# rlorenzo/facet

Hardware: AMD Instinct MI355X
Metric: images/sec whole-node (TOPIQ+SAMP+CLIP+InsightFace ensemble), 1024² batch (higher is better)
Workload: dtype f32

## Files before the change

facet_amd/csrc/engine.hip:

```cpp
#include "engine.h"
#include "onnx_graph.h"
#include "wino64_maps.h"
#include <algorithm>
#include <cmath>
#include <cstdlib>

namespace fe {

void WeightStore::set(const std::string& name, const float* data, const int64_t* shape, int ndim) {
  HostTensor h;
  h.shape.assign(shape, shape + ndim);
  h.data.assign(data, data + h.numel());
  t_[name] = std::move(h);
}
const HostTensor& WeightStore::get(const std::string& name) const {
  auto it = t_.find(name);
  if (it == t_.end()) throw Error("missing weight tensor '" + name + "'");
  return it->second;
}

float* DeviceWeights::upload(const std::vector<float>& v) {
  void* p = nullptr;
  const size_t b = v.size() * sizeof(float);
  FE_HIP(hipMalloc(&p, b ? b : 16));
// ... 663 lines not shown
}

template <class E>
static void linear_forward_half(Ctx& c, const ConvW& w, const E* x, int ldx, int M, E* y, int ldy, int act, const E* res, int ldr) {
  FE_CHECK(w.wh && w.hprec == PrecOf<E>::value, "linear(2-byte): layer has no weights of the activations' type");
  if (M <= 32 && !res && act != ACT_PRELU && ldx % 4 == 0 && ((uintptr_t)x & 7) == 0) {
    launch_gemm_skinny(x, ldx, (const E*)w.wh, w.KpH, w.scale, w.shift, y, ldy, M, w.Cout, w.CinPadH, act, c.stream);
    c.flops_accum += 2.0 * M * (double)w.Cin * (w.CoutAlg ? w.CoutAlg : w.Cout);
    return;
  }
  TensorT<E> xt = mat_view(x, M, w.CinPadH, ldx), yt = mat_view(y, M, w.Cout, ldy);
  ConvOptsT<E> o; o.act = act;
  TensorT<E> rt;
  if (res) { rt = mat_view(res, M, w.Cout, ldr); o.res = &rt; }
  conv_forward(c, w, xt, yt, o);
}
template <class E>
static void linear_forward_s32_half(Ctx& c, const ConvW& w, const E* x, int ldx, int M, float* y, int ldy, int act, const float* res, int ldr) {
  FE_CHECK(w.wh && w.hprec == PrecOf<E>::value, "linear(2-byte): layer has no weights of the activations' type");
  TensorT<E> xt = mat_view(x, M, w.CinPadH, ldx), yt = mat_view((E*)nullptr, M, w.Cout, 0);
  Tensor y32 = mat_view(y, M, w.Cout, ldy), r32;
  ConvOptsT<E> o; o.act = act; o.y32 = &y32;
  if (res) { r32 = mat_view(res, M, w.Cout, ldr); o.res32 = &r32; }
  conv_forward(c, w, xt, yt, o);
}
void linear_forward_s32(Ctx& c, const ConvW& w, const bf16* x, int ldx, int M, float* y, int ldy, int act, const float* res, int ldr) {
  linear_forward_s32_half<bf16>(c, w, x, ldx, M, y, ldy, act, res, ldr);
}
void linear_forward_s32(Ctx& c, const ConvW& w, const f16* x, int ldx, int M, float* y, int ldy, int act, const float* res, int ldr) {
  linear_forward_s32_half<f16>(c, w, x, ldx, M, y, ldy, act, res, ldr);
}
void linear_forward(Ctx& c, const ConvW& w, const bf16* x, int ldx, int M, bf16* y, int ldy, int act, const bf16* res, int ldr) {
  linear_forward_half<bf16>(c, w, x, ldx, M, y, ldy, act, res, ldr);
}
void linear_forward(Ctx& c, const ConvW& w, const f16* x, int ldx, int M, f16* y, int ldy, int act, const f16* res, int ldr) {
  linear_forward_half<f16>(c, w, x, ldx, M, y, ldy, act, res, ldr);
}
template <class E>
static void linear_forward_f32_half(Ctx& c, const ConvW& w, const E* x, int ldx, int M, float* y, int ldy, int act) {
  FE_CHECK(w.wh && w.hprec == PrecOf<E>::value && act != ACT_PRELU && ldx % 4 == 0 && ((uintptr_t)x & 7) == 0, "linear_f32(2-byte): unsupported layer");
  for (int m0 = 0; m0 < M; m0 += 32) {
    const int mb = std::min(32, M - m0);
    launch_gemm_skinny(x + (size_t)m0 * ldx, ldx, (const E*)w.wh, w.KpH, w.scale, w.shift, y + (size_t)m0 * ldy, ldy, mb, w.Cout, w.CinPadH, act, c.stream);
  }
  c.flops_accum += 2.0 * M * (double)w.Cin * (w.CoutAlg ? w.CoutAlg : w.Cout);
}
void linear_forward_f32(Ctx& c, const ConvW& w, const bf16* x, int ldx, int M, float* y, int ldy, int act) { linear_forward_f32_half<bf16>(c, w, x, ldx, M, y, ldy, act); }
void linear_forward_f32(Ctx& c, const ConvW& w, const f16* x, int ldx, int M, float* y, int ldy, int act) { linear_forward_f32_half<f16>(c, w, x, ldx, M, y, ldy, act); }
void linear_forward_xf32(Ctx& c, const ConvW& w, int prec, const float* x, int ldx, int M, float* y, int ldy, int act) {
  FE_CHECK(w.wh && w.hprec == prec && act != ACT_PRELU && ldx % 4 == 0 && ((uintptr_t)x & 15) == 0, "linear_xf32: unsupported layer");
  for (int m0 = 0; m0 < M; m0 += 32) {
    const int mb = std::min(32, M - m0);
    if (prec == PREC_F16) launch_gemm_skinny(x + (size_t)m0 * ldx, ldx, (const f16*)w.wh, w.KpH, w.scale, w.shift, y + (size_t)m0 * ldy, ldy, mb, w.Cout, w.CinPadH, act, c.stream);
    else launch_gemm_skinny(x + (size_t)m0 * ldx, ldx, (const bf16*)w.wh, w.KpH, w.scale, w.shift, y + (size_t)m0 * ldy, ldy, mb, w.Cout, w.CinPadH, act, c.stream);
  }
  c.flops_accum += 2.0 * M * (double)w.Cin * (w.CoutAlg ? w.CoutAlg : w.Cout);
}

MHAW build_mha(DeviceWeights& dw, const WeightStore& ws, const std::string& prefix, int heads) {
  MHAW m;
  const HostTensor& W = ws.get(prefix + ".in_proj_weight");
  const HostTensor& Bv = ws.get(prefix + ".in_proj_bias");
  const int d = (int)W.shape[1];
  FE_CHECK(W.shape[0] == 3 * d && d % heads == 0 && d % 32 == 0, "mha %s: bad in_proj shape", prefix.c_str());
  m.d = d; m.heads = heads;
  m.q = build_linear_rows(dw, W, nullptr, 0, d);
  m.k = build_linear_rows(dw, W, &Bv, d, d);
  const float sc = 1.0f / std::sqrt((float)(d / heads));
  std::vector<float> qs(d, sc), qb(d);
  for (int i = 0; i < d; ++i) qb[i] = Bv.data[i] * sc;
  m.q.scale = dw.upload(qs);
  m.q.shift = dw.upload(qb);
  std::vector<float> wv(W.data.begin() + (size_t)2 * d * d, W.data.begin() + (size_t)3 * d * d);
  std::vector<float> bv(Bv.data.begin() + 2 * d, Bv.data.begin() + 3 * d);
  m.wv = dw.upload(wv);
  m.bv = dw.upload(bv);
  if (dw.prec != PREC_F32) {
    std::vector<uint16_t> wvh(wv.size());
    for (size_t i = 0; i < wv.size(); ++i) wvh[i] = f32_to_half_bits(wv[i], dw.prec);
    m.wv_h = dw.upload_raw(wvh.data(), wvh.size() * sizeof(uint16_t));
  }
  m.out = build_linear(dw, ws, prefix + ".out_proj", true);
  return m;
}

static void launch_gemm(const ConvParams& p, hipStream_t s) { launch_conv(p, s); }
static void launch_gemm(const ConvParamsH& p, hipStream_t s) { launch_conv_bf16(p, s); }
static void launch_gemm(const ConvParamsT<f16>& p, hipStream_t s) { launch_conv_bf16(p, s); }

template <class T>
static void raw_gemm(Ctx& c, ConvParamsT<T>& p, double flops) {
  constexpr int kalign = sizeof(T) == 2 ? CONV_KALIGN_H : CONV_KALIGN;
  constexpr int valign = 16 / sizeof(T);
  p.N = 1; p.H = 1; p.W = p.M; p.Ho = 1; p.Wo = p.M;
  p.KH = p.KW = 1; p.sh = p.sw = p.dh = p.dw = 1; p.ph = p.pw = 0;
  p.Kp = (p.K + kalign - 1) / kalign * kalign;
  p.Cin = p.K;
  FE_CHECK(p.xs1 % valign == 0 && p.xs2 % valign == 0 && p.ws1 % valign == 0 && p.ws2 % valign == 0, "raw_gemm: batch strides must keep 16-B alignment");
  FE_CHECK(p.ldw == 0 || p.ldw == p.Kp || p.K % kalign == 0, "raw_gemm: K = %d must be a multiple of %d when the B operand is an activation matrix", p.K, kalign);
  hipEvent_t e0 = nullptr, e1 = nullptr;
  if (c.profile) {
    FE_HIP(hipEventCreate(&e0)); FE_HIP(hipEventCreate(&e1));
    FE_HIP(hipEventRecord(e0, c.stream));
  }
  launch_gemm(p, c.stream);
  if (c.profile) {
    FE_HIP(hipEventRecord(e1, c.stream));
    FE_HIP(hipEventSynchronize(e1));
    float ms = 0.f;
    FE_HIP(hipEventElapsedTime(&ms, e0, e1));
    (void)hipEventDestroy(e0); (void)hipEventDestroy(e1);
    char nm[128];
    snprintf(nm, sizeof nm, "%sbgemm x%d M=%d K=%d N=%d", PrecOf<T>::value == PREC_F16 ? "f16 " : (PrecOf<T>::value == PREC_BF16 ? "bf16 " : ""), p.batch > 1 ? p.batch : 1, p.M, p.K, p.Cout);
    c.timings.push_back({nm, flops, 0.0, ms});
  }
  c.flops_accum += flops;
  if (sizeof(T) == 2) c.flops_half += flops;
}

static const float* mha_wv(const MHAW& m, const float*) { return m.wv; }
static const bf16* mha_wv(const MHAW& m, const bf16*) {
  FE_CHECK(m.wv_h && m.q.hprec == PREC_BF16, "mha(bf16): model was not committed under bf16 precision");
  return (const bf16*)m.wv_h;
}
static const f16* mha_wv(const MHAW& m, const f16*) {
  FE_CHECK(m.wv_h && m.q.hprec == PREC_F16, "mha(f16): model was not committed under f16 precision");
  return (const f16*)m.wv_h;
}

void linear_forward_res(Ctx& c, const ConvW& w, const float* x, int ldx, int M, float* y, int ldy, int act, const float* res, int ldr) { linear_forward(c, w, x, ldx, M, y, ldy, act, res, ldr); }
void linear_forward_res(Ctx& c, const ConvW& w, const bf16* x, int ldx, int M, bf16* y, int ldy, int act, const bf16* res, int ldr) { linear_forward(c, w, x, ldx, M, y, ldy, act, res, ldr); }
void linear_forward_res(Ctx& c, const ConvW& w, const f16* x, int ldx, int M, f16* y, int ldy, int act, const f16* res, int ldr) { linear_forward(c, w, x, ldx, M, y, ldy, act, res, ldr); }
void linear_forward_res(Ctx& c, const ConvW& w, const bf16* x, int ldx, int M, float* y, int ldy, int act, const float* res, int ldr) { linear_forward_s32(c, w, x, ldx, M, y, ldy, act, res, ldr); }
void linear_forward_res(Ctx& c, const ConvW& w, const f16* x, int ldx, int M, float* y, int ldy, int act, const float* res, int ldr) { linear_forward_s32(c, w, x, ldx, M, y, ldy, act, res, ldr); }

template <class T, class RT>
void mha_forward(Ctx& c, const MHAW& m, const T* q_in, int ldq, const T* kv_in, int ldkv, int B, int Lq, int Lk,
                 const RT* res, int ldr, RT* y, int ldy, bool causal) {
  constexpr bool half = sizeof(T) == 2;
  const int d = m.d, H = m.heads, hd = d / H;
  const int Lp = (Lk + 31) / 32 * 32;
  const size_t mark = c.arena.mark();
  T* Q = c.arena.array<T>((size_t)B * Lq * d);
  T* K = c.arena.array<T>((size_t)B * Lk * d);
  T* Vt = c.arena.array<T>((size_t)B * d * Lp);
  static const bool no_flash = getenv("FE_NO_FLASH") != nullptr;
  const bool flash = (hd == 64) && (!no_flash || half);
  FE_CHECK(flash || !causal, "causal attention needs the fused kernel (head_dim 64)");
  FE_CHECK(flash || !half, "attention(bf16) needs head_dim 64");
  T* S = flash ? nullptr : c.arena.array<T>((size_t)B * H * Lq * Lp);
  T* O = c.arena.array<T>((size_t)B * Lq * d);
  linear_forward(c, m.q, q_in, ldq, B * Lq, Q, d, ACT_NONE);
  linear_forward(c, m.k, kv_in, ldkv, B * Lk, K, d, ACT_NONE);
  if (Lp != Lk) FE_HIP(hipMemsetAsync(Vt, 0, (size_t)B * d * Lp * sizeof(T), c.stream));
  {
    ConvParamsT<T> p{};
    p.x = mha_wv(m, q_in); p.ldx = d; p.w = kv_in; p.ldw = ldkv; p.y = Vt; p.ldy = Lp;
    p.M = d; p.K = d; p.Cout = Lk;
    p.batch = B; p.nb1 = 1; p.ws2 = (long long)Lk * ldkv; p.ys2 = (long long)d * Lp;
    p.pad_store = half ? 1 : 0;
    raw_gemm(c, p, 2.0 * B * d * (double)d * Lk);
  }
  if (flash) {
    launch_attention(Q, d, K, d, Vt, Lp, m.bv, O, d, B, H, Lq, Lk, d, causal ? 1 : 0, c.stream);
    c.flops_accum += 4.0 * B * H * (double)Lq * Lk * hd;
    if (half) c.flops_half += 4.0 * B * H * (double)Lq * Lk * hd;
  } else if constexpr (!half) {
    {
      ConvParams p{};
      p.x = Q; p.ldx = d; p.w = K; p.ldw = d; p.y = S; p.ldy = Lp;
      p.M = Lq; p.K = hd; p.Cout = Lk;
      p.batch = B * H; p.nb1 = H;
      p.xs1 = hd; p.xs2 = (long long)Lq * d; p.ws1 = hd; p.ws2 = (long long)Lk * d;
      p.ys1 = (long long)Lq * Lp; p.ys2 = (long long)H * Lq * Lp;
      raw_gemm(c, p, 2.0 * B * H * (double)Lq * Lk * hd);
    }
    launch_softmax_rows_pad(S, Lp, B * H * Lq, Lk, c.stream);
    {
      ConvParams p{};
      p.x = S; p.ldx = Lp; p.w = Vt; p.ldw = Lp; p.y = O; p.ldy = d;
      p.shift = m.bv; p.hs1 = hd;
      p.M = Lq; p.K = Lp; p.Cout = hd;
      p.batch = B * H; p.nb1 = H;
      p.xs1 = (long long)Lq * Lp; p.xs2 = (long long)H * Lq * Lp;
      p.ws1 = (long long)hd * Lp; p.ws2 = (long long)d * Lp;
      p.ys1 = hd; p.ys2 = (long long)Lq * d;
      raw_gemm(c, p, 2.0 * B * H * (double)Lq * Lk * hd);
    }
  }
  linear_forward_res(c, m.out, (const T*)O, d, B * Lq, y, ldy, ACT_NONE, res, ldr);
  c.arena.rewind(mark);
}
template void mha_forward<float, float>(Ctx&, const MHAW&, const float*, int, const float*, int, int, int, int, const float*, int, float*, int, bool);
template void mha_forward<bf16, bf16>(Ctx&, const MHAW&, const bf16*, int, const bf16*, int, int, int, int, const bf16*, int, bf16*, int, bool);
template void mha_forward<f16, f16>(Ctx&, const MHAW&, const f16*, int, const f16*, int, int, int, int, const f16*, int, f16*, int, bool);
template void mha_forward<bf16, float>(Ctx&, const MHAW&, const bf16*, int, const bf16*, int, int, int, int, const float*, int, float*, int, bool);
template void mha_forward<f16, float>(Ctx&, const MHAW&, const f16*, int, const f16*, int, int, int, int, const float*, int, float*, int, bool);

}
```

facet_amd/csrc/fe_common.h:

```cpp
#pragma once
#include <hip/hip_runtime.h>
#include "fe_check.h"
#include <cstdint>
#include <cstdio>
#include <atomic>
#include <cstring>
#include <map>
#include <mutex>
#include <stdexcept>
#include <string>
#include <utility>
#include <vector>

namespace fe {


#define FE_HIP(expr)                                                                      \
  do {                                                                                    \
    hipError_t _e = (expr);                                                               \
    if (_e != hipSuccess) {                                                               \
      char _b[512];                                                                       \
      snprintf(_b, sizeof _b, "%s:%d: %s -> %s", __FILE__, __LINE__, #expr,               \
               hipGetErrorString(_e));                                                    \
      throw fe::Error(_b);                                                                \
// ... 163 lines not shown
    return (char*)base_ + a;
  }
  template <class T>
  TensorT<T> tensor_t(int n, int h, int w, int c) {
    TensorT<T> t;
    t.n = n; t.h = h; t.w = w; t.c = c; t.ld = c;
    t.p = (T*)alloc(t.numel() * sizeof(T));
    return t;
  }
  Tensor tensor(int n, int h, int w, int c) { return tensor_t<float>(n, h, w, c); }
  template <class T>
  T* array(size_t count) { return (T*)alloc(count * sizeof(T)); }
 private:
  void* base_ = nullptr;
  size_t cap_ = 0, off_ = 0, high_ = 0;
};

template <class T>
struct ConvParamsT {
  const T* x; int ldx;
  const T* w;
  const float* scale;
  const float* shift;
  const float* slope;
  const T* res; int ldr;
  const T* gate; int ldg;
  T* y; int ldy;
  int N, H, W, Cin, Ho, Wo, Cout;
  int KH, KW, sh, sw, ph, pw, dh, dw;
  int K, Kp, M;
  int act;
  int res_after_act;
  int gate_c1;
  int vec_epi;
  int unit_stride;
  int ldw;
  int batch, nb1;
  long long xs1, xs2, ws1, ws2, ys1, ys2, hs1;
  int buf_ok; unsigned x_span, w_span;
  unsigned y_span, r_span, g_span;
  int variant;
  int cb;
  int pad_store;
  const float* res32; int ldr32;
  float* y32; int ldy32;
  unsigned r32_span, y32_span;
  int a_wrap;
  int split_lo_off;
  int exact_act;
};
using ConvParams = ConvParamsT<float>;
using ConvParamsH = ConvParamsT<bf16>;

struct ConvW {
  float* w = nullptr;
  float* scale = nullptr;
  float* shift = nullptr;
  float* slope = nullptr;
  int Cout = 0, Cin = 0, CinPad = 0, KH = 1, KW = 1, K = 0, Kp = 0;
  int CoutAlg = 0;
  float* wtap = nullptr;
  int wino_m = 0;
  float* wino = nullptr;
  float* wino64 = nullptr;
  float* wstem = nullptr;
  float* wn16 = nullptr;
  int KpT = 0;
  void* wh = nullptr;
  int hprec = 0;
  int KpH = 0, cb = 0, CinPadH = 0;
  void* wtap_h = nullptr;
  int KpTH = 0;
  uint8_t* w8 = nullptr;
  float* w8_scale = nullptr;
};

template <class T>
struct ConvOptsT {
  int sh = 1, sw = 1, ph = 0, pw = 0, dh = 1, dw = 1;
  int act = ACT_NONE;
  const TensorT<T>* res = nullptr;
  int res_after_act = 0;
  const TensorT<T>* gate = nullptr;
  const TensorT<float>* res32 = nullptr;
  const TensorT<float>* y32 = nullptr;
};
using ConvOpts = ConvOptsT<float>;

constexpr int CONV_KALIGN = 32;
constexpr int CONV_KALIGN_H = 64;

void launch_conv(const ConvParams& p, hipStream_t s);
void launch_wino_input(const Tensor& x, int th, int tw, float* V, hipStream_t s);
void launch_wino_output(const float* Mb, const Tensor& y, int th, int tw, const float* scale, const float* shift, int relu, hipStream_t s);
void launch_wino4_input(const Tensor& x, int th, int tw, float* V, hipStream_t s);
void launch_wino4_output(const float* Mb, const Tensor& y, int th, int tw, const float* scale, const float* shift, int act, const float* slope,
                         const Tensor* res, int res_after_act, hipStream_t s);
void launch_wino64(const Tensor& x, const Tensor& y, const float* U, const float* scale, const float* shift, const float* slope, int act,
                   const Tensor* res, int res_after_act, hipStream_t s);
template <class TO>
bool launch_stem(const float* x, int ldx, int N, int H, int W, const float* wstem, const float* scale, const float* shift, const float* slope,
                 int Cout, int k, int stride, int act, TO* y, int ldy, int Ho, int Wo, hipStream_t s);
void launch_conv_narrow(const ConvParams& p, hipStream_t s);
void launch_conv_dma(const ConvParams& p, int tile, hipStream_t s);
void launch_conv_bf16(const ConvParamsH& p, hipStream_t s);
void launch_conv_bf16(const ConvParamsT<f16>& p, hipStream_t s);
template <class T, class Launch>
inline bool conv_split_by_images(const ConvParamsT<T>& p, Launch&& launch) {
  if (p.batch > 1 || p.N <= 1 || (long long)p.N * p.Ho * p.Wo != (long long)p.M) return false;
  const unsigned long long in_img = (unsigned long long)p.H * p.W * p.ldx * sizeof(T);
  unsigned long long out_img = (unsigned long long)p.Ho * p.Wo * (unsigned long long)(p.ldy > p.ldr ? p.ldy : p.ldr) * sizeof(T);
  const unsigned long long out32_img = (unsigned long long)p.Ho * p.Wo * (unsigned long long)(p.ldy32 > p.ldr32 ? p.ldy32 : p.ldr32) * sizeof(float);
  if ((p.y32 || p.res32) && out32_img > out_img) out_img = out32_img;
  const unsigned long long per_img = in_img > out_img ? in_img : out_img;
  constexpr unsigned long long LIMIT = 0xF0000000ull;
  if (per_img >= LIMIT) return false;
  const int ng = (int)(LIMIT / per_img);
  if (ng >= p.N) return false;
  for (int i0 = 0; i0 < p.N; i0 += ng) {
    ConvParamsT<T> q = p;
    const int n = ng < p.N - i0 ? ng : p.N - i0;
    const size_t opix = (size_t)i0 * p.Ho * p.Wo;
    q.N = n; q.M = n * p.Ho * p.Wo;
    q.x = p.x + (size_t)i0 * p.H * p.W * p.ldx;
    if (p.y) q.y = p.y + opix * p.ldy;
    if (p.y32) q.y32 = p.y32 + opix * p.ldy32;
    if (p.res32) q.res32 = p.res32 + opix * p.ldr32;
    if (p.res) q.res = p.res + opix * p.ldr;
    if (p.gate) q.gate = p.gate + opix * p.ldg;
    launch(q);
  }
  return true;
}

double conv_flops(const ConvParams& p);

void launch_u8_to_nhwc4_norm(const uint8_t* src, float* dst, size_t pixels, const float mean[3],
                             const float stdv[3], int bgr, hipStream_t s);
template <class T> void launch_nchw_to_nhwc(const float* src, T* dst, int n, int c, int h, int w, int cpad, hipStream_t s);
template <class T> void launch_nhwc_to_nchw(const T* src, int lds_, float* dst, int n, int c, int h, int w, hipStream_t s);
template <class T> void launch_maxpool(const TensorT<T>& x, const TensorT<T>& y, int k, int stride, int pad, hipStream_t s);
template <class T> void launch_bilinear(const TensorT<T>& x, const TensorT<T>& y, hipStream_t s);
template <class T> void launch_adaptive_avgpool(const TensorT<T>& x, const TensorT<T>& y, hipStream_t s);
void launch_convert(const float* x, bf16* y, size_t n, hipStream_t s);
void launch_convert(const bf16* x, float* y, size_t n, hipStream_t s);
void launch_convert(const float* x, f16* y, size_t n, hipStream_t s);
void launch_convert(const f16* x, float* y, size_t n, hipStream_t s);
void launch_splitk_reduce(const float* part, int splits, int M, int N, const float* scale, const float* shift, const float* slope, int act,
                          const float* res, int ldr, int res_after_act, float* y, int ldy, hipStream_t s);
template <class T>
void launch_tap_gather(const T* z, int ldz, int n, int h, int w, int kh, int kw, int ph, int pw, int dh, int dw,
                       int cout, const float* scale, const float* shift, int act, T* y, int ldy, int ho, int wo,
                       hipStream_t s);
void launch_attention(const float* q, int ldq, const float* k, int ldk, const float* vt, int lp, const float* bv, float* o,
                      int ldo, int B, int H, int Lq, int Lk, int dmodel, int causal, hipStream_t s);
void launch_attention(const bf16* q, int ldq, const bf16* k, int ldk, const bf16* vt, int lp, const float* bv, bf16* o,
                      int ldo, int B, int H, int Lq, int Lk, int dmodel, int causal, hipStream_t s);
void launch_attention(const f16* q, int ldq, const f16* k, int ldk, const f16* vt, int lp, const float* bv, f16* o,
                      int ldo, int B, int H, int Lq, int Lk, int dmodel, int causal, hipStream_t s);
void launch_attention_split(const f16* q, const f16* k, int ld, int lo_off, const f16* vt_hi, const f16* vt_lo, int lp, f16* o, int ldo, int o_lo_off,
                            int B, int H, int Lq, int Lk, int dmodel, hipStream_t s);
template <class TI, class TW, class TO>
void launch_gemm_skinny(const TI* x, int ldx, const TW* w, int ldw, const float* scale, const float* shift, TO* y,
                        int ldy, int M, int N, int K, int act, hipStream_t s);
void launch_sigmoid(const Tensor& x, const Tensor& y, hipStream_t s);
void launch_add(const Tensor& a, const Tensor& b, const Tensor& y, hipStream_t s);
void launch_layernorm_split(const float* x, int ldx, f16* y, int ldy, const float* g, const float* b, int rows, int d, float eps, hipStream_t s);
void launch_split_hi_lo(const float* x, f16* y, size_t rows, int cols, hipStream_t s);
template <class T, class TO>
void launch_layernorm(const T* x, int ldx, TO* y, int ldy, const float* g, const float* b,
                      int rows, int d, float eps, hipStream_t s);
void launch_softmax_rows(float* x, int ld, int rows, int d, hipStream_t s);
void launch_softmax_rows_pad(float* x, int ld, int rows, int d, hipStream_t s);
template <class T>
void launch_add_rows_bcast(T* y, int ldy, const float* pos, int rows, int L, int d, hipStream_t s);

void launch_affine_act(const Tensor& x, const Tensor& y, const float* scale, const float* shift, int act, const float* slope,
                       hipStream_t s);
void launch_binary(const Tensor& a, const Tensor& b, const Tensor& y, int op, int act, hipStream_t s);
void launch_gather_strided(const float* src, float* dst, const long long dims[6], const long long sstr[6], hipStream_t s);
void launch_nearest(const Tensor& x, const Tensor& y, hipStream_t s);
void launch_avgpool(const Tensor& x, const Tensor& y, int k, int stride, int pad, int include_pad, hipStream_t s);
void launch_dwconv(const Tensor& x, const Tensor& y, const float* wt, int kh, int kw, int sh, int sw, int ph, int pw,
                   const float* scale, const float* shift, int act, const float* slope, const Tensor* res, hipStream_t s);

void launch_cv_resize_linear(const uint8_t* src, int n, int h, int w, uint8_t* dst, int ch, int cw, int nh, int nw, const int* xofs,
                             const short* ialpha, const int* yofs, const short* ibeta, int area2, hipStream_t s);
void launch_warp_affine(const uint8_t* src, int h, int w, const int* img_of, const double* Minv, int m, int S, const short* wtab,
                        uint8_t* dst, hipStream_t s);
void launch_swap_rb_u8(const uint8_t* src, uint8_t* dst, size_t pixels, hipStream_t s);
void launch_u8_blob(const uint8_t* src, float* dst, size_t pixels, float mean, float scale, int swap_rb, hipStream_t s);
void launch_scrfd_decode(const float* scores, const float* bbox, const float* kps, int n, int fh, int fw, int A, int K, int stride,
                         float thresh, float det_scale, int level, float* cand, int* counts, int max_cand, hipStream_t s);
void cv_resize_tables(int src, int dst, bool clamp_fx, std::vector<int>& ofs, std::vector<short>& coef);
void cv_warp_weight_table(std::vector<short>& wtab);

constexpr int FE_STATS_COUNT = 264;
size_t stats_accum_bytes(int n);
void launch_image_stats(const uint8_t* bgr, int n, int h, int w, uint8_t* gray, uint8_t* hsv_out, const int* sdiv, const int* hdiv, void* accum,
                        double* out, hipStream_t s);
void cv_hsv_tables(std::vector<int>& sdiv, std::vector<int>& hdiv);
void launch_roi_laplacian(const uint8_t* bgr, int h, int w, const int* img_of, const int* rois, int m, double* out, hipStream_t s);
void launch_canny_map(const uint8_t* d_bgr, int n, int h, int w, int low, int high, uint8_t* d_blur, void* d_grad, void* d_mag, uint8_t* d_map,
                      hipStream_t s);
void launch_canny_map_gray(const uint8_t* d_gray, int n, int h, int w, const int* d_thr, void* d_grad, void* d_mag, uint8_t* d_map, hipStream_t s);
struct ContourScratch {
  int* lab_fg;
  int* lab_bg;
  int* cnt;
  int* strong;
  int* xmin;
  int* xmax;
  int* ymax;
  uint8_t* outer;
  uint8_t* edge;
  int* work;
  int* work_count;
  long long* recs;
  int* rec_count;
  int* error;
};
constexpr int FE_CONTOUR_RECORD = 8;
int contour_work_cap(int h, int w);
size_t contour_scratch_bytes(int nb, int h, int w);
void contour_scratch_carve(ContourScratch& sc, void* base, int nb, int h, int w);
void launch_median_thresholds(const double* d_stats, int n, long long npx, int* d_thr, hipStream_t s);
void launch_external_contours(const uint8_t* d_img, int nb, int h, int w, int candidates, long long min_twice_area, ContourScratch& sc,
                              hipStream_t s);

}
```

facet_amd/csrc/kernels_attn.hip:

```cpp
#include <type_traits>

#include "fe_common.h"

namespace fe {

template <class T>
struct AttnParamsH {
  const T* q; int ldq;
  const T* k; int ldk;
  const T* vt; int lp;
  const float* bv;
  T* o; int ldo;
  int B, H, Lq, Lk, dmodel;
  int causal;
};
struct AttnParams : AttnParamsH<float> {};
struct AttnSplitParams {
  const f16* q; const f16* k; int ld; int lo_off;
  const f16* vt_hi; const f16* vt_lo; int lp;
  f16* o; int ldo; int o_lo_off;
  int B, H, Lq, Lk, dmodel;
};

template <class T>
struct AttnLds {
  static constexpr int KS = 64 * sizeof(T) + 16;
  static constexpr int VS = sizeof(T) == 4 ? 144 : 72;
  static constexpr int K_BYTES = 32 * KS, V_BYTES = 64 * VS;
};
template <class T, int NT>
struct AttnStage {
  typedef unsigned U4 __attribute__((ext_vector_type(4)));
  typedef unsigned U2 __attribute__((ext_vector_type(2)));
  using V4 = std::conditional_t<sizeof(T) == 4, U4, U2>;
  static constexpr int KE = 16 / sizeof(T), KC = 64 / KE;
  static constexpr int KN = 32 * KC / NT, VN = 64 * 8 / NT;
  const T* Kp; int ldk;
  const T* Vp; int lp;
  U4 kr[KN];
  V4 vr[VN];
  __device__ __forceinline__ void load(int kt, int Lk, int t) {
#pragma unroll
    for (int i = 0; i < KN; ++i) {
      const int c = t + i * NT;
      int row = kt * 32 + c / KC;
      if (row > Lk - 1) row = Lk - 1;
      kr[i] = *reinterpret_cast<const U4*>(Kp + (size_t)row * ldk + (c % KC) * KE);
    }
#pragma unroll
    for (int i = 0; i < VN; ++i) {
      const int c = t + i * NT;
      vr[i] = *reinterpret_cast<const V4*>(Vp + (size_t)(c >> 3) * lp + kt * 32 + (c & 7) * 4);
    }
  }
  __device__ __forceinline__ void store(char* Ks, char* Vs, int t) const {
#pragma unroll
    for (int i = 0; i < KN; ++i) { const int c = t + i * NT; *reinterpret_cast<U4*>(&Ks[(c / KC) * AttnLds<T>::KS + (c % KC) * 16]) = kr[i]; }
#pragma unroll
    for (int i = 0; i < VN; ++i) { const int c = t + i * NT; *reinterpret_cast<V4*>(&Vs[(c >> 3) * AttnLds<T>::VS + (c & 7) * sizeof(V4)]) = vr[i]; }
  }
};

template <class T, class ParamsT>
struct AttnDense {
  using Params = ParamsT;
  static constexpr int K_BYTES = AttnLds<T>::K_BYTES, V_BYTES = AttnLds<T>::V_BYTES;
  static __device__ __forceinline__ bool causal(const Params& p) { return p.causal; }
  static __device__ __forceinline__ float ex(float x) { return __expf(x); }
  static __device__ __forceinline__ const T* q_row(const Params& p, int b, int head, int qc) {
    return p.q + (size_t)b * p.Lq * p.ldq + head * 64 + (size_t)qc * p.ldq;
  }
  template <int NT>
  static __device__ __forceinline__ AttnStage<T, NT> stage(const Params& p, int b, int head) {
    return {p.k + (size_t)b * p.Lk * p.ldk + head * 64, p.ldk, p.vt + ((size_t)b * p.dmodel + head * 64) * p.lp, p.lp};
  }
  static __device__ __forceinline__ void write(const Params& p, int b, int head, int q, int h, const fe_f32x16& o0, const fe_f32x16& o1, float inv) {
    T* op = p.o + ((size_t)b * p.Lq + q) * p.ldo + head * 64;
    const float* bp = p.bv + head * 64;
#pragma unroll
    for (int g = 0; g < 4; ++g) {
      const int d0 = 8 * g + 4 * h;
      const float4 b0 = *reinterpret_cast<const float4*>(bp + d0);
      const float4 b1 = *reinterpret_cast<const float4*>(bp + 32 + d0);
      st4(op + d0, make_float4(o0[4 * g] * inv + b0.x, o0[4 * g + 1] * inv + b0.y, o0[4 * g + 2] * inv + b0.z, o0[4 * g + 3] * inv + b0.w));
      st4(op + 32 + d0, make_float4(o1[4 * g] * inv + b1.x, o1[4 * g + 1] * inv + b1.y, o1[4 * g + 2] * inv + b1.z, o1[4 * g + 3] * inv + b1.w));
    }
  }
};

struct AttnF32 : AttnDense<float, AttnParams> {
  struct Q {
    float4 f[8];
    __device__ __forceinline__ void load(const Params& p, int b, int head, int qc, int h) {
#pragma unroll
      for (int s = 0; s < 8; ++s) f[s] = *reinterpret_cast<const float4*>(q_row(p, b, head, qc) + 8 * s + 4 * h);
    }
  };
  static __device__ __forceinline__ fe_f32x16 scores(const char* Ks, const Q& q, int r, int h) {
    fe_f32x16 st;
#pragma unroll
    for (int e = 0; e < 16; ++e) st[e] = 0.f;
    const char* kb = &Ks[r * AttnLds<float>::KS + 16 * h];
#pragma unroll
    for (int s = 0; s < 8; ++s) {
      const float4 kf = *reinterpret_cast<const float4*>(kb + 32 * s);
      st = __builtin_amdgcn_mfma_f32_32x32x2f32(kf.x, q.f[s].x, st, 0, 0, 0);
      st = __builtin_amdgcn_mfma_f32_32x32x2f32(kf.y, q.f[s].y, st, 0, 0, 0);
      st = __builtin_amdgcn_mfma_f32_32x32x2f32(kf.z, q.f[s].z, st, 0, 0, 0);
      st = __builtin_amdgcn_mfma_f32_32x32x2f32(kf.w, q.f[s].w, st, 0, 0, 0);
    }
    return st;
  }
  static __device__ __forceinline__ void pv(fe_f32x16& o0, fe_f32x16& o1, const fe_f32x16& st, const char* Vs, int r, int h) {
    const char* vb = &Vs[r * AttnLds<float>::VS + 16 * h];
#pragma unroll
    for (int g = 0; g < 4; ++g) {
      const float4 v0 = *reinterpret_cast<const float4*>(vb + 32 * g);
      const float4 v1 = *reinterpret_cast<const float4*>(vb + 32 * AttnLds<float>::VS + 32 * g);
      o0 = __builtin_amdgcn_mfma_f32_32x32x2f32(v0.x, st[4 * g + 0], o0, 0, 0, 0);
      o1 = __builtin_amdgcn_mfma_f32_32x32x2f32(v1.x, st[4 * g + 0], o1, 0, 0, 0);
      o0 = __builtin_amdgcn_mfma_f32_32x32x2f32(v0.y, st[4 * g + 1], o0, 0, 0, 0);
      o1 = __builtin_amdgcn_mfma_f32_32x32x2f32(v1.y, st[4 * g + 1], o1, 0, 0, 0);
      o0 = __builtin_amdgcn_mfma_f32_32x32x2f32(v0.z, st[4 * g + 2], o0, 0, 0, 0);
      o1 = __builtin_amdgcn_mfma_f32_32x32x2f32(v1.z, st[4 * g + 2], o1, 0, 0, 0);
      o0 = __builtin_amdgcn_mfma_f32_32x32x2f32(v0.w, st[4 * g + 3], o0, 0, 0, 0);
      o1 = __builtin_amdgcn_mfma_f32_32x32x2f32(v1.w, st[4 * g + 3], o1, 0, 0, 0);
    }
  }
};

union AttnF8 { uint4 u; fe_v4f f; };
struct AttnQ8 {
  AttnF8 f[4];
  template <class E>
  __device__ __forceinline__ void load(const E* row, int h) {
#pragma unroll
    for (int s = 0; s < 4; ++s) f[s].u = *reinterpret_cast<const uint4*>(row + 16 * s + 8 * h);
  }
};
static __device__ __forceinline__ fe_v4f attn_k8(const char* kb, int s) {
  AttnF8 k;
  k.u = *reinterpret_cast<const uint4*>(kb + 32 * s);
  return k.f;
}
static __device__ __forceinline__ fe_v4f attn_v8(const char* vb, int s) {
  const uint2 a0 = *reinterpret_cast<const uint2*>(vb + 32 * s), a1 = *reinterpret_cast<const uint2*>(vb + 32 * s + 16);
  AttnF8 v;
  v.u = make_uint4(a0.x, a0.y, a1.x, a1.y);
  return v.f;
}
template <class E>
static __device__ __forceinline__ fe_v4f attn_p8(const E* tag, const fe_f32x16& x, int s) {
  AttnF8 pf;
  pf.u = make_uint4(fe_pack2(tag, x[8 * s], x[8 * s + 1]), fe_pack2(tag, x[8 * s + 2], x[8 * s + 3]),
                    fe_pack2(tag, x[8 * s + 4], x[8 * s + 5]), fe_pack2(tag, x[8 * s + 6], x[8 * s + 7]));
  return pf.f;
}

template <class E>
struct AttnHalf : AttnDense<E, AttnParamsH<E>> {
  using Params = AttnParamsH<E>;
  struct Q : AttnQ8 {
    __device__ __forceinline__ void load(const Params& p, int b, int head, int qc, int h) { AttnQ8::load(AttnHalf::q_row(p, b, head, qc), h); }
  };
  static __device__ __forceinline__ fe_f32x16 scores(const char* Ks, const Q& q, int r, int h) {
    const E* const tag = nullptr;
    fe_f32x16 st;
#pragma unroll
    for (int e = 0; e < 16; ++e) st[e] = 0.f;
    const char* kb = &Ks[r * AttnLds<f16>::KS + 16 * h];
#pragma unroll
    for (int s = 0; s < 4; ++s) st = fe_mfma16(tag, attn_k8(kb, s), q.f[s].f, st);
    return st;
  }
  static __device__ __forceinline__ void pv(fe_f32x16& o0, fe_f32x16& o1, const fe_f32x16& st, const char* Vs, int r, int h) {
    const E* const tag = nullptr;
    const char* vb = &Vs[r * AttnLds<f16>::VS + 8 * h];
#pragma unroll
    for (int s = 0; s < 2; ++s) {
      const fe_v4f pf = attn_p8(tag, st, s);
      o0 = fe_mfma16(tag, attn_v8(vb, s), pf, o0);
      o1 = fe_mfma16(tag, attn_v8(vb + 32 * AttnLds<f16>::VS, s), pf, o1);
    }
  }
};

struct AttnSplit {
  using Params = AttnSplitParams;
  using L = AttnLds<f16>;
  static constexpr int K_BYTES = 2 * L::K_BYTES, V_BYTES = 2 * L::V_BYTES;
  static __device__ __forceinline__ bool causal(const Params&) { return false; }
  static __device__ __forceinline__ float ex(float x) { return expf(x); }
  struct Q {
    AttnQ8 hi, lo;
    __device__ __forceinline__ void load(const Params& p, int b, int head, int qc, int h) {
      const f16* row = p.q + (size_t)b * p.Lq * p.ld + head * 64 + (size_t)qc * p.ld;
      hi.load(row, h);
      lo.load(row + p.lo_off, h);
    }
  };
  template <int NT>
  struct Stage {
    AttnStage<f16, NT> hi, lo;
    __device__ __forceinline__ void load(int kt, int Lk, int t) { hi.load(kt, Lk, t); lo.load(kt, Lk, t); }
    __device__ __forceinline__ void store(char* Ks, char* Vs, int t) const {
      hi.store(Ks, Vs, t);
      lo.store(Ks + L::K_BYTES, Vs + L::V_BYTES, t);
    }
  };
  template <int NT>
  static __device__ __forceinline__ Stage<NT> stage(const Params& p, int b, int head) {
    const f16* Kp = p.k + (size_t)b * p.Lk * p.ld + head * 64;
    const size_t v0 = ((size_t)b * p.dmodel + head * 64) * p.lp;
    return {{Kp, p.ld, p.vt_hi + v0, p.lp}, {Kp + p.lo_off, p.ld, p.vt_lo + v0, p.lp}};
  }
  static __device__ __forceinline__ fe_f32x16 scores(const char* Ks, const Q& q, int r, int h) {
    const f16* const tag = nullptr;
    fe_f32x16 st;
#pragma unroll
    for (int e = 0; e < 16; ++e) st[e] = 0.f;
    const char* kb = &Ks[r * AttnLds<f16>::KS + 16 * h];
#pragma unroll
    for (int s = 0; s < 4; ++s) {
      const fe_v4f kh = attn_k8(kb, s), kl = attn_k8(kb + L::K_BYTES, s);
      st = fe_mfma16(tag, kl, q.hi.f[s].f, st);
      st = fe_mfma16(tag, kh, q.lo.f[s].f, st);
      st = fe_mfma16(tag, kh, q.hi.f[s].f, st);
    }
    return st;
  }
  static __device__ __forceinline__ void pv(fe_f32x16& o0, fe_f32x16& o1, const fe_f32x16& st, const char* Vs, int r, int h) {
    const f16* const tag = nullptr;
    const char* vb = &Vs[r * L::VS + 8 * h];
    fe_f32x16 lo;
#pragma unroll
    for (int e = 0; e < 16; ++e) lo[e] = st[e] - (float)fe_to_f16(st[e]);
#pragma unroll
    for (int s = 0; s < 2; ++s) {
      const fe_v4f ph = attn_p8(tag, st, s), pl = attn_p8(tag, lo, s);
      const fe_v4f v0h = attn_v8(vb, s), v1h = attn_v8(vb + 32 * L::VS, s);
      const fe_v4f v0l = attn_v8(vb + L::V_BYTES, s), v1l = attn_v8(vb + L::V_BYTES + 32 * L::VS, s);
      o0 = fe_mfma16(tag, v0l, ph, o0); o0 = fe_mfma16(tag, v0h, pl, o0); o0 = fe_mfma16(tag, v0h, ph, o0);
      o1 = fe_mfma16(tag, v1l, ph, o1); o1 = fe_mfma16(tag, v1h, pl, o1); o1 = fe_mfma16(tag, v1h, ph, o1);
    }
  }
  static __device__ __forceinline__ void write(const Params& p, int b, int head, int q, int h, const fe_f32x16& o0, const fe_f32x16& o1, float inv) {
    f16* op = p.o + ((size_t)b * p.Lq + q) * p.ldo + head * 64;
#pragma unroll
    for (int g = 0; g < 4; ++g) {
      const int d0 = 8 * g + 4 * h;
      const float4 a = make_float4(o0[4 * g] * inv, o0[4 * g + 1] * inv, o0[4 * g + 2] * inv, o0[4 * g + 3] * inv);
      const float4 c = make_float4(o1[4 * g] * inv, o1[4 * g + 1] * inv, o1[4 * g + 2] * inv, o1[4 * g + 3] * inv);
      const float4 ah = make_float4((float)fe_to_f16(a.x), (float)fe_to_f16(a.y), (float)fe_to_f16(a.z), (float)fe_to_f16(a.w));
      const float4 ch = make_float4((float)fe_to_f16(c.x), (float)fe_to_f16(c.y), (float)fe_to_f16(c.z), (float)fe_to_f16(c.w));
      st4(op + d0, ah); st4(op + 32 + d0, ch);
      st4(op + p.o_lo_off + d0, make_float4(a.x - ah.x, a.y - ah.y, a.z - ah.z, a.w - ah.w));
      st4(op + p.o_lo_off + 32 + d0, make_float4(c.x - ch.x, c.y - ch.y, c.z - ch.z, c.w - ch.w));
    }
  }
};

template <class P, int NW>
__device__ __forceinline__ void attn_fwd_body(const typename P::Params& p) {
  __shared__ __attribute__((aligned(16))) char Ks[2][P::K_BYTES];
  __shared__ __attribute__((aligned(16))) char Vs[2][P::V_BYTES];
  const int t = threadIdx.x, lane = t & 63, wave = t >> 6;
  const int r = lane & 31, h = lane >> 5;
  const int bh = blockIdx.y, b = bh / p.H, head = bh - b * p.H;
  const int q = (blockIdx.x * NW + wave) * 32 + r;
  const bool qok = q < p.Lq;
  typename P::Q qf;
  qf.load(p, b, head, qok ? q : p.Lq - 1, h);
  auto stage = P::template stage<NW * 64>(p, b, head);

  fe_f32x16 o0, o1;
#pragma unroll
  for (int e = 0; e < 16; ++e) { o0[e] = 0.f; o1[e] = 0.f; }
  float m = -INFINITY, l = 0.f;

  const int nt = (p.Lk + 31) / 32;
  stage.load(0, p.Lk, t);
  stage.store(Ks[0], Vs[0], t);
  __syncthreads();
  for (int kt = 0; kt < nt; ++kt) {
    const int buf = kt & 1;
    if (kt + 1 < nt) stage.load(kt + 1, p.Lk, t);
    fe_f32x16 st = P::scores(Ks[buf], qf, r, h);
    const int kbase = kt * 32 + 4 * h;
    float tmax = -INFINITY;
#pragma unroll
    for (int e = 0; e < 16; ++e) {
      const int key = kbase + (e & 3) + 8 * (e >> 2);
      if (key >= p.Lk || (P::causal(p) && key > q)) st[e] = -INFINITY;
      tmax = fmaxf(tmax, st[e]);
    }
    tmax = fmaxf(tmax, __shfl_xor(tmax, 32));
    const float mn = fmaxf(m, tmax);
    const float alpha = P::ex(m - mn);
    float psum = 0.f;
#pragma unroll
    for (int e = 0; e < 16; ++e) { st[e] = P::ex(st[e] - mn); psum += st[e]; }
    psum += __shfl_xor(psum, 32);
    l = l * alpha + psum;
    m = mn;
#pragma unroll
    for (int e = 0; e < 16; ++e) { o0[e] *= alpha; o1[e] *= alpha; }
    P::pv(o0, o1, st, Vs[buf], r, h);
    if (kt + 1 < nt) stage.store(Ks[buf ^ 1], Vs[buf ^ 1], t);
    __syncthreads();
  }
  if (qok) P::write(p, b, head, q, h, o0, o1, 1.f / l);
}

template <int NW>
__global__ __launch_bounds__(NW * 64, 2) void attn_fwd_kernel(const AttnParams p) { attn_fwd_body<AttnF32, NW>(p); }
template <class E, int NW>
__global__ __launch_bounds__(NW * 64, 2) void attn_fwd_bf16_kernel(const AttnParamsH<E> p) { attn_fwd_body<AttnHalf<E>, NW>(p); }
template <int NW>
__global__ __launch_bounds__(NW * 64, 2) void attn_fwd_split_kernel(const AttnSplitParams p) { attn_fwd_body<AttnSplit, NW>(p); }

template <class Params>
static void attn_launch(void (*k4)(Params), void (*k2)(Params), const Params& p, hipStream_t s) {
  const int w4 = (p.Lq + 127) / 128 * 128, w2 = (p.Lq + 63) / 64 * 64;
  if (k2 == nullptr || w4 * 100 <= w2 * 108) {
    hipLaunchKernelGGL(k4, dim3((p.Lq + 127) / 128, p.B * p.H), dim3(256), 0, s, p);
  } else {
    hipLaunchKernelGGL(k2, dim3((p.Lq + 63) / 64, p.B * p.H), dim3(128), 0, s, p);
  }
  FE_HIP(hipGetLastError());
}

void launch_attention(const float* q, int ldq, const float* k, int ldk, const float* vt, int lp, const float* bv, float* o,
                      int ldo, int B, int H, int Lq, int Lk, int dmodel, int causal, hipStream_t s) {
  FE_CHECK(dmodel == H * 64, "attention kernel is built for head_dim 64 (d_model %d, %d heads)", dmodel, H);
  FE_CHECK(ldq % 4 == 0 && ldk % 4 == 0 && lp % 4 == 0 && ldo % 4 == 0 && lp >= (Lk + 31) / 32 * 32, "attention: strides");
  FE_CHECK((((uintptr_t)q | (uintptr_t)k | (uintptr_t)vt | (uintptr_t)bv | (uintptr_t)o) & 15) == 0, "attention: alignment");
  const AttnParams p{{q, ldq, k, ldk, vt, lp, bv, o, ldo, B, H, Lq, Lk, dmodel, causal}};
  attn_launch<AttnParams>(attn_fwd_kernel<4>, attn_fwd_kernel<2>, p, s);
}

template <class E>
static void launch_attention_half(const E* q, int ldq, const E* k, int ldk, const E* vt, int lp, const float* bv, E* o,
                                  int ldo, int B, int H, int Lq, int Lk, int dmodel, int causal, hipStream_t s) {
  FE_CHECK(dmodel == H * 64, "attention kernel is built for head_dim 64 (d_model %d, %d heads)", dmodel, H);
  FE_CHECK(ldq % 8 == 0 && ldk % 8 == 0 && lp % 4 == 0 && ldo % 4 == 0 && lp >= (Lk + 31) / 32 * 32, "attention(2-byte): strides");
  FE_CHECK((((uintptr_t)q | (uintptr_t)k | (uintptr_t)bv) & 15) == 0 && (((uintptr_t)vt | (uintptr_t)o) & 7) == 0, "attention(2-byte): alignment");
  const AttnParamsH<E> p{q, ldq, k, ldk, vt, lp, bv, o, ldo, B, H, Lq, Lk, dmodel, causal};
  attn_launch<AttnParamsH<E>>(attn_fwd_bf16_kernel<E, 4>, attn_fwd_bf16_kernel<E, 2>, p, s);
}
void launch_attention(const bf16* q, int ldq, const bf16* k, int ldk, const bf16* vt, int lp, const float* bv, bf16* o,
                      int ldo, int B, int H, int Lq, int Lk, int dmodel, int causal, hipStream_t s) {
  launch_attention_half(q, ldq, k, ldk, vt, lp, bv, o, ldo, B, H, Lq, Lk, dmodel, causal, s);
}
void launch_attention(const f16* q, int ldq, const f16* k, int ldk, const f16* vt, int lp, const float* bv, f16* o,
                      int ldo, int B, int H, int Lq, int Lk, int dmodel, int causal, hipStream_t s) {
  launch_attention_half(q, ldq, k, ldk, vt, lp, bv, o, ldo, B, H, Lq, Lk, dmodel, causal, s);
}

void launch_attention_split(const f16* q, const f16* k, int ld, int lo_off, const f16* vt_hi, const f16* vt_lo, int lp, f16* o, int ldo, int o_lo_off,
                            int B, int H, int Lq, int Lk, int dmodel, hipStream_t s) {
  FE_CHECK(dmodel == H * 64 && ld % 8 == 0 && lo_off % 8 == 0 && lp % 4 == 0 && ldo % 4 == 0 && o_lo_off % 4 == 0 && lp >= (Lk + 31) / 32 * 32, "attention(split): geometry");
  FE_CHECK((((uintptr_t)q | (uintptr_t)k) & 15) == 0 && (((uintptr_t)vt_hi | (uintptr_t)vt_lo | (uintptr_t)o) & 7) == 0, "attention(split): alignment");
  const AttnSplitParams p{q, k, ld, lo_off, vt_hi, vt_lo, lp, o, ldo, o_lo_off, B, H, Lq, Lk, dmodel};
  attn_launch<AttnSplitParams>(attn_fwd_split_kernel<4>, nullptr, p, s);
}

}
```

Measured before the change: 237.3.

## Handle short attention key tails with scalar path and skip idle waves

For f32 and split-f16 attention, when the key length leaves a remainder of at most four keys beyond a 32-key tile, those keys are now staged into small shared arrays and handled with scalar dot products instead of a whole padded MFMA tile. Waves whose query block is entirely out of range skip compute, and the per-element masking runs only on boundary or causal tiles. The V padding memset now clears only the pad columns and is skipped when the kernel does not read them. The 2-wave vs 4-wave launch choice becomes a simple Lq threshold. This adds register/shared usage and scalar code that may be slower than the MFMA path for some shapes.

```diff
diff --git a/facet_amd/csrc/engine.hip b/facet_amd/csrc/engine.hip
--- a/facet_amd/csrc/engine.hip
+++ b/facet_amd/csrc/engine.hip
@@ -839,7 +839,8 @@
   T* O = c.arena.array<T>((size_t)B * Lq * d);
   linear_forward(c, m.q, q_in, ldq, B * Lq, Q, d, ACT_NONE);
   linear_forward(c, m.k, kv_in, ldkv, B * Lk, K, d, ACT_NONE);
-  if (Lp != Lk) FE_HIP(hipMemsetAsync(Vt, 0, (size_t)B * d * Lp * sizeof(T), c.stream));
+  if (Lp != Lk && (!flash || attention_reads_vt_pad(Lk, half)))
+    FE_HIP(hipMemset2DAsync(Vt + Lk, (size_t)Lp * sizeof(T), 0, (size_t)(Lp - Lk) * sizeof(T), (size_t)B * d, c.stream));
   {
     ConvParamsT<T> p{};
     p.x = mha_wv(m, q_in); p.ldx = d; p.w = kv_in; p.ldw = ldkv; p.y = Vt; p.ldy = Lp;
diff --git a/facet_amd/csrc/fe_common.h b/facet_amd/csrc/fe_common.h
--- a/facet_amd/csrc/fe_common.h
+++ b/facet_amd/csrc/fe_common.h
@@ -339,6 +339,8 @@
 void launch_tap_gather(const T* z, int ldz, int n, int h, int w, int kh, int kw, int ph, int pw, int dh, int dw,
                        int cout, const float* scale, const float* shift, int act, T* y, int ldy, int ho, int wo,
                        hipStream_t s);
+constexpr int ATTN_TAIL = 4;
+inline bool attention_reads_vt_pad(int Lk, bool two_byte) { return Lk % 32 > (two_byte ? 0 : ATTN_TAIL); }
 void launch_attention(const float* q, int ldq, const float* k, int ldk, const float* vt, int lp, const float* bv, float* o,
                       int ldo, int B, int H, int Lq, int Lk, int dmodel, int causal, hipStream_t s);
 void launch_attention(const bf16* q, int ldq, const bf16* k, int ldk, const bf16* vt, int lp, const float* bv, bf16* o,
diff --git a/facet_amd/csrc/kernels_attn.hip b/facet_amd/csrc/kernels_attn.hip
--- a/facet_amd/csrc/kernels_attn.hip
+++ b/facet_amd/csrc/kernels_attn.hip
@@ -89,6 +89,17 @@
 };
 
 struct AttnF32 : AttnDense<float, AttnParams> {
+  static constexpr int TAIL = ATTN_TAIL;
+  template <int NT>
+  static __device__ __forceinline__ void stage_tail(const Params& p, int b, int head, int base, int tail, float (*Kt)[64], float (*Vt)[64], int t) {
+    const float* Kp = p.k + ((size_t)b * p.Lk + base) * p.ldk + head * 64;
+    const float* Vp = p.vt + ((size_t)b * p.dmodel + head * 64) * p.lp + base;
+    for (int i = t; i < tail * 64; i += NT) {
+      const int j = i >> 6, c = i & 63;
+      Kt[j][c] = Kp[(size_t)j * p.ldk + c];
+      Vt[j][c] = Vp[(size_t)c * p.lp + j];
+    }
+  }
   struct Q {
     float4 f[8];
     __device__ __forceinline__ void load(const Params& p, int b, int head, int qc, int h) {
@@ -110,6 +121,15 @@
       st = __builtin_amdgcn_mfma_f32_32x32x2f32(kf.w, q.f[s].w, st, 0, 0, 0);
     }
     return st;
+  }
+  static __device__ __forceinline__ float tail_dot(const Q& q, const float* krow, int h) {
+    float acc = 0.f;
+#pragma unroll
+    for (int s = 0; s < 8; ++s) {
+      const float4 kf = *reinterpret_cast<const float4*>(krow + 8 * s + 4 * h);
+      acc = fmaf(kf.x, q.f[s].x, acc); acc = fmaf(kf.y, q.f[s].y, acc); acc = fmaf(kf.z, q.f[s].z, acc); acc = fmaf(kf.w, q.f[s].w, acc);
+    }
+    return acc;
   }
   static __device__ __forceinline__ void pv(fe_f32x16& o0, fe_f32x16& o1, const fe_f32x16& st, const char* Vs, int r, int h) {
     const char* vb = &Vs[r * AttnLds<float>::VS + 16 * h];
@@ -137,6 +157,20 @@
 #pragma unroll
     for (int s = 0; s < 4; ++s) f[s].u = *reinterpret_cast<const uint4*>(row + 16 * s + 8 * h);
   }
+  template <class E>
+  __device__ __forceinline__ float tail_dot(const E* tag, const float* krow, int h) const {
+    float acc = 0.f;
+#pragma unroll
+    for (int s = 0; s < 4; ++s) {
+      const float4 k0 = *reinterpret_cast<const float4*>(krow + 16 * s + 8 * h), k1 = *reinterpret_cast<const float4*>(krow + 16 * s + 8 * h + 4);
+      float a, b;
+      fe_unpack2(tag, f[s].u.x, a, b); acc = fmaf(k0.x, a, acc); acc = fmaf(k0.y, b, acc);
+      fe_unpack2(tag, f[s].u.y, a, b); acc = fmaf(k0.z, a, acc); acc = fmaf(k0.w, b, acc);
+      fe_unpack2(tag, f[s].u.z, a, b); acc = fmaf(k1.x, a, acc); acc = fmaf(k1.y, b, acc);
+      fe_unpack2(tag, f[s].u.w, a, b); acc = fmaf(k1.z, a, acc); acc = fmaf(k1.w, b, acc);
+    }
+    return acc;
+  }
 };
 static __device__ __forceinline__ fe_v4f attn_k8(const char* kb, int s) {
   AttnF8 k;
@@ -160,6 +194,7 @@
 template <class E>
 struct AttnHalf : AttnDense<E, AttnParamsH<E>> {
   using Params = AttnParamsH<E>;
+  static constexpr int TAIL = 0;
   struct Q : AttnQ8 {
     __device__ __forceinline__ void load(const Params& p, int b, int head, int qc, int h) { AttnQ8::load(AttnHalf::q_row(p, b, head, qc), h); }
   };
@@ -189,6 +224,7 @@
   using Params = AttnSplitParams;
   using L = AttnLds<f16>;
   static constexpr int K_BYTES = 2 * L::K_BYTES, V_BYTES = 2 * L::V_BYTES;
+  static constexpr int TAIL = ATTN_TAIL;
   static __device__ __forceinline__ bool causal(const Params&) { return false; }
   static __device__ __forceinline__ float ex(float x) { return expf(x); }
   struct Q {
@@ -213,6 +249,20 @@
     const f16* Kp = p.k + (size_t)b * p.Lk * p.ld + head * 64;
     const size_t v0 = ((size_t)b * p.dmodel + head * 64) * p.lp;
     return {{Kp, p.ld, p.vt_hi + v0, p.lp}, {Kp + p.lo_off, p.ld, p.vt_lo + v0, p.lp}};
+  }
+  template <int NT>
+  static __device__ __forceinline__ void stage_tail(const Params& p, int b, int head, int base, int tail, float (*Kt)[64], float (*Vt)[64], int t) {
+    const f16* Kp = p.k + ((size_t)b * p.Lk + base) * p.ld + head * 64;
+    const size_t v0 = ((size_t)b * p.dmodel + head * 64) * p.lp + base;
+    for (int i = t; i < tail * 64; i += NT) {
+      const int j = i >> 6, c = i & 63;
+      Kt[j][c] = (float)Kp[(size_t)j * p.ld + c] + (float)Kp[(size_t)j * p.ld + p.lo_off + c];
+      Vt[j][c] = (float)p.vt_hi[v0 + (size_t)c * p.lp + j] + (float)p.vt_lo[v0 + (size_t)c * p.lp + j];
+    }
+  }
+  static __device__ __forceinline__ float tail_dot(const Q& q, const float* krow, int h) {
+    const f16* const tag = nullptr;
+    return q.lo.tail_dot(tag, krow, h) + q.hi.tail_dot(tag, krow, h);
   }
   static __device__ __forceinline__ fe_f32x16 scores(const char* Ks, const Q& q, int r, int h) {
     const f16* const tag = nullptr;
@@ -260,14 +310,28 @@
   }
 };
 
+static __device__ __forceinline__ void attn_tail_pv(fe_f32x16& o0, fe_f32x16& o1, float pj, const float* vrow, int h) {
+#pragma unroll
+  for (int g = 0; g < 4; ++g) {
+    const float4 v0 = *reinterpret_cast<const float4*>(vrow + 8 * g + 4 * h), v1 = *reinterpret_cast<const float4*>(vrow + 32 + 8 * g + 4 * h);
+    o0[4 * g] = fmaf(pj, v0.x, o0[4 * g]); o0[4 * g + 1] = fmaf(pj, v0.y, o0[4 * g + 1]);
+    o0[4 * g + 2] = fmaf(pj, v0.z, o0[4 * g + 2]); o0[4 * g + 3] = fmaf(pj, v0.w, o0[4 * g + 3]);
+    o1[4 * g] = fmaf(pj, v1.x, o1[4 * g]); o1[4 * g + 1] = fmaf(pj, v1.y, o1[4 * g + 1]);
+    o1[4 * g + 2] = fmaf(pj, v1.z, o1[4 * g + 2]); o1[4 * g + 3] = fmaf(pj, v1.w, o1[4 * g + 3]);
+  }
+}
+
 template <class P, int NW>
 __device__ __forceinline__ void attn_fwd_body(const typename P::Params& p) {
   __shared__ __attribute__((aligned(16))) char Ks[2][P::K_BYTES];
   __shared__ __attribute__((aligned(16))) char Vs[2][P::V_BYTES];
-  const int t = threadIdx.x, lane = t & 63, wave = t >> 6;
+  constexpr int TAIL = P::TAIL;
+  __shared__ __attribute__((aligned(16))) float Kt[TAIL ? TAIL : 1][64], Vt[TAIL ? TAIL : 1][64];
+  const int t = threadIdx.x, lane = t & 63, wave = __builtin_amdgcn_readfirstlane(t >> 6);
   const int r = lane & 31, h = lane >> 5;
   const int bh = blockIdx.y, b = bh / p.H, head = bh - b * p.H;
-  const int q = (blockIdx.x * NW + wave) * 32 + r;
+  const int q0 = (blockIdx.x * NW + wave) * 32, q = q0 + r;
+  const bool live = q0 < p.Lq;
   const bool qok = q < p.Lq;
   typename P::Q qf;
   qf.load(p, b, head, qok ? q : p.Lq - 1, h);
@@ -278,36 +342,77 @@
   for (int e = 0; e < 16; ++e) { o0[e] = 0.f; o1[e] = 0.f; }
   float m = -INFINITY, l = 0.f;
 
-  const int nt = (p.Lk + 31) / 32;
-  stage.load(0, p.Lk, t);
-  stage.store(Ks[0], Vs[0], t);
+  const int tail = p.Lk & 31;
+  const bool vtail = tail >= 1 && tail <= TAIL;
+  const int nt = p.Lk / 32 + (tail > TAIL ? 1 : 0);
+  if (nt > 0) {
+    stage.load(0, p.Lk, t);
+    stage.store(Ks[0], Vs[0], t);
+  }
+  if constexpr (TAIL > 0) {
+    if (vtail) P::template stage_tail<NW * 64>(p, b, head, nt * 32, tail, Kt, Vt, t);
+  }
   __syncthreads();
   for (int kt = 0; kt < nt; ++kt) {
     const int buf = kt & 1;
     if (kt + 1 < nt) stage.load(kt + 1, p.Lk, t);
-    fe_f32x16 st = P::scores(Ks[buf], qf, r, h);
-    const int kbase = kt * 32 + 4 * h;
-    float tmax = -INFINITY;
-#pragma unroll
-    for (int e = 0; e < 16; ++e) {
-      const int key = kbase + (e & 3) + 8 * (e >> 2);
-      if (key >= p.Lk || (P::causal(p) && key > q)) st[e] = -INFINITY;
-      tmax = fmaxf(tmax, st[e]);
-    }
-    tmax = fmaxf(tmax, __shfl_xor(tmax, 32));
-    const float mn = fmaxf(m, tmax);
-    const float alpha = P::ex(m - mn);
-    float psum = 0.f;
-#pragma unroll
-    for (int e = 0; e < 16; ++e) { st[e] = P::ex(st[e] - mn); psum += st[e]; }
-    psum += __shfl_xor(psum, 32);
-    l = l * alpha + psum;
-    m = mn;
-#pragma unroll
-    for (int e = 0; e < 16; ++e) { o0[e] *= alpha; o1[e] *= alpha; }
-    P::pv(o0, o1, st, Vs[buf], r, h);
+    if (live) {
+      fe_f32x16 st = P::scores(Ks[buf], qf, r, h);
+      const int kbase = kt * 32 + 4 * h;
+      if (kt * 32 + 32 > p.Lk || (P::causal(p) && kt * 32 + 31 > q0)) {
+#pragma unroll
+        for (int e = 0; e < 16; ++e) {
+          const int key = kbase + (e & 3) + 8 * (e >> 2);
+          if (key >= p.Lk || (P::causal(p) && key > q)) st[e] = -INFINITY;
+        }
+      }
+      float tmax = -INFINITY;
+#pragma unroll
+      for (int e = 0; e < 16; ++e) tmax = fmaxf(tmax, st[e]);
+      tmax = fmaxf(tmax, __shfl_xor(tmax, 32));
+      const float mn = fmaxf(m, tmax);
+      const float alpha = P::ex(m - mn);
+      float psum = 0.f;
+#pragma unroll
+      for (int e = 0; e < 16; ++e) { st[e] = P::ex(st[e] - mn); psum += st[e]; }
+      psum += __shfl_xor(psum, 32);
+      l = l * alpha + psum;
+      m = mn;
+#pragma unroll
+      for (int e = 0; e < 16; ++e) { o0[e] *= alpha; o1[e] *= alpha; }
+      P::pv(o0, o1, st, Vs[buf], r, h);
+    }
     if (kt + 1 < nt) stage.store(Ks[buf ^ 1], Vs[buf ^ 1], t);
     __syncthreads();
+  }
+  if constexpr (TAIL > 0) {
+    if (vtail && live) {
+      float sc[TAIL], tmax = -INFINITY;
+#pragma unroll
+      for (int j = 0; j < TAIL; ++j) {
+        sc[j] = -INFINITY;
+        if (j < tail) {
+          const float d = P::tail_dot(qf, Kt[j], h);
+          sc[j] = d + __shfl_xor(d, 32);
+          if (P::causal(p) && nt * 32 + j > q) sc[j] = -INFINITY;
+          tmax = fmaxf(tmax, sc[j]);
+        }
+      }
+      const float mn = fmaxf(m, tmax);
+      const float alpha = P::ex(m - mn);
+#pragma unroll
+      for (int e = 0; e < 16; ++e) { o0[e] *= alpha; o1[e] *= alpha; }
+      float psum = 0.f;
+#pragma unroll
+      for (int j = 0; j < TAIL; ++j) {
+        if (j < tail) {
+          const float pj = P::ex(sc[j] - mn);
+          psum += pj;
+          attn_tail_pv(o0, o1, pj, Vt[j], h);
+        }
+      }
+      l = l * alpha + psum;
+    }
   }
   if (qok) P::write(p, b, head, q, h, o0, o1, 1.f / l);
 }
@@ -321,8 +426,7 @@
 
 template <class Params>
 static void attn_launch(void (*k4)(Params), void (*k2)(Params), const Params& p, hipStream_t s) {
-  const int w4 = (p.Lq + 127) / 128 * 128, w2 = (p.Lq + 63) / 64 * 64;
-  if (k2 == nullptr || w4 * 100 <= w2 * 108) {
+  if (k2 == nullptr || p.Lq > 64) {
     hipLaunchKernelGGL(k4, dim3((p.Lq + 127) / 128, p.B * p.H), dim3(256), 0, s, p);
   } else {
     hipLaunchKernelGGL(k2, dim3((p.Lq + 63) / 64, p.B * p.H), dim3(128), 0, s, p);
```

Result: no change. 237.7 (median of 2 runs) (+0.2%).
